# Vill-Lab/2023-TIFS-ISTVT

Measured on AMD Instinct MI355X. Metric: clips/sec (BxTx3x224x224 fwd+bwd), higher is better.
Workload: dtype bf16; 1 GPU; C2: B=32/GPU T=8 224x224 full ISTVT (Xception stem + 12-layer DSTTr) train step (fwd+bwd+grad all-reduce+SGD), random-init weights; global_batch=32, frames=8, size=224, depth=12, parallelism=dp1, early_allreduce=False, attn_fp8=False, dead_row_elimination=False, final_norm_class_rows_only=False, optimizer=SGD(momentum 0.9) fused, step_graphs=False

## Files before the change

### 2023-tifs-istvt_amd/_lib.py

```python
import ctypes
import os
from ctypes import c_float, c_int, c_long, c_void_p

_HERE = os.path.dirname(os.path.abspath(__file__))
LIB_PATH = os.environ.get('ISTVT_LIB') or os.path.join(_HERE, 'libistvt_hip.so')

P, I, L, F = c_void_p, c_int, c_long, c_float


class JpegDecodeArgs(ctypes.Structure):
    _fields_ = [('bytes', P), ('nbytes', L), ('images', P), ('images_host', P), ('segments', P), ('segments_host', P),
                ('qtabs', P), ('htabs', P), ('scratch', P), ('scratch_bytes', L), ('out', P), ('sizes', P), ('status', P),
                ('stream', P), ('n', I), ('nseg', I), ('nq', I), ('nh', I), ('Hc', I), ('Wc', I)]


class JpegEncodeArgs(ctypes.Structure):
    _fields_ = [('frames', P), ('total', L), ('quality', P), ('header', P), ('header_bytes', L), ('scratch', P),
                ('scratch_bytes', L), ('data', P), ('capacity', L), ('offsets', P), ('status', P), ('stream', P), ('n', I),
                ('H', I), ('W', I), ('subsampling', I), ('restart_interval', I), ('dqt0', I), ('dqt1', I)]


SIGNATURES = {
    'istvt_gemm': [P, L, I, P, L, I, P, L, I, I, I, P, P, L, P, I, I, I, F, P, P, I, I, P],
    'istvt_layernorm_fwd': [P, L, P, P, P, L, P, P, L, I, F, I, P],
# ... 11 lines not shown
    'istvt_attn_spatial_relevance': [P, L, P, L, P, P, P, I, I, I, I, F, I, P],
    'istvt_attn_temporal_relevance': [P, L, P, L, P, P, I, I, I, I, I, F, I, I, P],
    'istvt_relevance_heatmap': [P, P, I, I, I, P],
    'istvt_relevance_fuse_windows': [P, P, P, P, P, P, P, P, P, I, I, I, I, I, I, P],
    'istvt_relevance_overlay_u8': [P, P, P, P, P, I, I, I, I, P],
    'istvt_windows_reduce': [P, P, P, P, I, I, I, P],
    'istvt_auc_pairs': [P, P, F, P, L, P, P, I, P],
    'istvt_tokens_fwd': [P, P, P, P, P, L, I, I, I, I, I, I, P],
    'istvt_tokens_gather_fwd': [P, P, P, P, P, P, L, I, I, I, I, I, I, I, P],
    'istvt_tokens_bwd': [P, L, P, P, P, P, P, I, I, I, I, I, I, P],
    'istvt_frame_diff': [P, P, I, I, I, I, I, I, P],
    'istvt_stats_replicas': [],
    'istvt_stats_reduce': [P, I, P],
    'istvt_stats_reduce_add': [P, I, P, P],
    'istvt_bn_stats': [P, P, P, L, I, I, P],
    'istvt_bn_finalize': [P, P, ctypes.c_double, P, P, P, P, F, F, P, I, I, I, P],
    'istvt_bn_apply': [P, P, P, L, I, I, I, P],
    'istvt_bn_bwd_stats': [P, P, P, P, P, L, I, I, P],
    'istvt_bn_bwd_apply': [P, P, P, P, P, P, P, P, P, L, I, I, I, P],
    'istvt_bn_add_fwd': [P, P, P, P, P, L, I, I, P],
    'istvt_pw_bwd': [P, P, P, P, P, P, P, L, P, L, P, P, P, P, P, L, I, I, I, I, P],
    'istvt_pw_bwd_grid': [L],
    'istvt_pw_bwd_rows': [],
    'istvt_im2col_conv1': [P, P, I, I, I, P],
    'istvt_conv1_fwd': [P, P, P, I, I, I, P],
    'istvt_conv1_fwd_u8': [P, P, P, P, P, I, I, I, P],
    'istvt_conv1_wgrad': [P, P, P, P, I, I, I, P],
    'istvt_conv1_wgrad_slabs': [],
    'istvt_conv1_fwd_u8_view': [P, L, I, I, P, P, P, P, P, I, I, I, P],
    'istvt_conv1_wgrad_u8': [P, P, L, I, I, P, P, P, P, P, I, I, I, P],
    'istvt_im2col_conv1_u8': [P, L, I, I, P, P, P, P, I, I, I, P],
    'istvt_crop_resize_u8': [P, L, I, I, P, P, I, I, P],
    'istvt_crop_resize_nv12': [P, L, I, I, L, L, P, P, P, I, I, P],
    'istvt_nv12_to_rgb_u8': [P, L, I, I, L, L, P, P, I, P],
    'istvt_warp_similarity_u8': [P, L, I, I, P, P, I, I, P],
    'istvt_warp_similarity_nv12': [P, L, I, I, L, L, P, P, P, I, I, P],
    'istvt_relevance_paste_u8': [P, L, I, I, P, I, P, P, P, P, I, I, P],
    'istvt_relevance_paste_nv12': [P, L, I, I, L, L, P, I, P, P, P, P, I, I, P],
    'istvt_jpeg_roundtrip_u8': [P, L, I, I, I, P, I, P, L, P, P],
    'istvt_jpeg_decode_u8': [ctypes.POINTER(JpegDecodeArgs)],
    'istvt_jpeg_decode_split_u8': [ctypes.POINTER(JpegDecodeArgs), I],
    'istvt_jpeg_decode_indexed_u8': [ctypes.POINTER(JpegDecodeArgs), I, I, I, I, I],
    'istvt_jpeg_decode_indexed_split_u8': [ctypes.POINTER(JpegDecodeArgs), I, I, I, I, I, I, I, I],
    'istvt_batch_draw': [ctypes.POINTER(JpegDecodeArgs), I, I, I],
    'istvt_jpeg_decode_drawn_u8': [ctypes.POINTER(JpegDecodeArgs), I, I, I, I, I, I, I],
    'istvt_jpeg_decode_drawn_split_u8': [ctypes.POINTER(JpegDecodeArgs), I, I, I, I, I, I, I, I, I, I],
# ... 88 lines not shown
```

### 2023-tifs-istvt_amd/csrc/pw_bwd.hip

```cpp
#include "common.h"
#include "bn_bwd.h"

constexpr int PW_R = 128;
constexpr int PW_THREADS = 512;

__host__ __device__ constexpr int pw_lds_row(int p) { return (p & ~31) | ((p & 4) << 2) | ((p & 24) >> 1) | (p & 3); }

static inline int pw_bwd_split(long M, long* kper_out) {
    long splits = M / 512 < 1 ? 1 : (M / 512 > 256 ? 256 : M / 512);
    if (splits > (M + 63) / 64) splits = (M + 63) / 64;
    long kper = (M + splits - 1) / splits;
    kper = (kper + 63) / 64 * 64;
    if (kper_out) *kper_out = kper;
    return (int)((M + kper - 1) / kper);
}

template <int CIN, int COUT>
struct PwTile {
    static constexpr int NU = PW_R * (COUT / 8) / PW_THREADS;
    static constexpr int ND = PW_R * (CIN / 8) / PW_THREADS;
    bf16x8 dz[NU], u[NU], d[ND];
};

template <int CIN, int COUT>
__global__ __launch_bounds__(PW_THREADS) void pw_bwd_kernel(
    const bf16_t* __restrict__ dz, const bf16_t* __restrict__ u, const float* __restrict__ bnp,
    const float* __restrict__ gamma, const double* s1, const double* s2, const bf16_t* __restrict__ d, long ldd,
    const bf16_t* __restrict__ wt, long ldwt, bf16_t* __restrict__ dd, float* __restrict__ ws, float* dgamma,
    float* dbeta, long M, long kper, int batch_stats) {
    static_assert(COUT == 128 && (CIN == 64 || CIN == 128), "instantiated shapes");
    constexpr int LDU = COUT + 16, LDD = CIN + 16;
    constexpr int UCH = COUT / 8, DCH = CIN / 8;
    constexpr int UROWS = PW_THREADS / UCH, DROWS = PW_THREADS / DCH;
    constexpr int KT = CIN / 16, KS = COUT / 32;
    constexpr int MT = (PW_R / 16) * KT / 8;
    typedef PwTile<CIN, COUT> Tile;
    __shared__ __attribute__((aligned(16))) bf16_t s_du[PW_R * LDU];
    __shared__ __attribute__((aligned(16))) bf16_t s_d[PW_R * LDD];
    __shared__ __attribute__((aligned(16))) bf16_t s_dd[PW_R * LDD];
    __shared__ __attribute__((aligned(16))) BnBwdChunk s_kc[UCH];

    const int tid = threadIdx.x, lane = tid & 63;
    const int wave = __builtin_amdgcn_readfirstlane(tid >> 6);
    const int g = lane >> 4, r = lane & 15;
    const long row_begin = (long)blockIdx.x * kper;
    const long row_end = min(M, row_begin + kper);
    const long nblk = (row_end - row_begin + PW_R - 1) / PW_R;

    const int uc = tid % UCH, ur = tid / UCH;
    const int dc = tid % DCH, dr = tid / DCH;
    const float invM = batch_stats ? 1.0f / (float)M : 0.0f;
    if (tid < UCH) bn_bwd_chunk_load(s_kc[tid], bnp, gamma, s1, s2, COUT, tid * 8, invM);
    __syncthreads();

    const int kt_dd = wave % KT, mt0 = (wave / KT) * MT;
    bf16x8 wf[KS];
#pragma unroll
    for (int s = 0; s < KS; ++s)
        wf[s] = *reinterpret_cast<const bf16x8*>(wt + (long)(kt_dd * 16 + r) * ldwt + s * 32 + g * 8);

    f32x4 accw[KT];
#pragma unroll
    for (int kt = 0; kt < KT; ++kt) accw[kt] = f32x4{0.f, 0.f, 0.f, 0.f};

    constexpr unsigned OOB = 0x80000000u, RSRC_FLAGS = 0x00020000u;
    const __amdgpu_buffer_rsrc_t dz_rs = __builtin_amdgcn_make_buffer_rsrc((void*)dz, 0, (int)(row_end * COUT * 2), RSRC_FLAGS);
    const __amdgpu_buffer_rsrc_t u_rs = __builtin_amdgcn_make_buffer_rsrc((void*)u, 0, (int)(row_end * COUT * 2), RSRC_FLAGS);
    const __amdgpu_buffer_rsrc_t d_rs = __builtin_amdgcn_make_buffer_rsrc((void*)d, 0, (int)(row_end * ldd * 2), RSRC_FLAGS);
    const __amdgpu_buffer_rsrc_t dd_rs = __builtin_amdgcn_make_buffer_rsrc((void*)dd, 0, (int)(row_end * CIN * 2), RSRC_FLAGS);
    const int ldd2 = (int)ldd * 2;

    auto load = [&](Tile& t, const long b) {
        const long row0 = row_begin + b * PW_R;
#pragma unroll
        for (int i = 0; i < Tile::NU; ++i) {
            const long row = row0 + ur + i * UROWS;
            const unsigned off = row < row_end ? (unsigned)((int)row * (COUT * 2) + uc * 16) : OOB;
            t.dz[i] = __builtin_bit_cast(bf16x8, __builtin_amdgcn_raw_buffer_load_b128(dz_rs, off, 0, 0));
            t.u[i] = __builtin_bit_cast(bf16x8, __builtin_amdgcn_raw_buffer_load_b128(u_rs, off, 0, 0));
        }
#pragma unroll
        for (int i = 0; i < Tile::ND; ++i) {
            const long row = row0 + dr + i * DROWS;
            const unsigned off = row < row_end ? (unsigned)((int)row * ldd2 + dc * 16) : OOB;
            t.d[i] = __builtin_bit_cast(bf16x8, __builtin_amdgcn_raw_buffer_load_b128(d_rs, off, 0, 0));
        }
    };

    auto block = [&](Tile& t, const long b, const long bnext) {
        const long row0 = row_begin + b * PW_R;
        const BnBwdChunk kc = s_kc[uc];
#pragma unroll
        for (int i = 0; i < Tile::NU; ++i) {
            const int lr = ur + i * UROWS;
            const unsigned keep = row0 + lr < row_end ? 0xffffffffu : 0u;
            bf16x8 o;
#pragma unroll
            for (int j = 0; j < 8; ++j) o[j] = (bf16_t)bn_bwd_du((float)t.dz[i][j], (float)t.u[i][j], kc, j);
            *reinterpret_cast<u32x4*>(s_du + pw_lds_row(lr) * LDU + uc * 8) = __builtin_bit_cast(u32x4, o) & keep;
        }
#pragma unroll
        for (int i = 0; i < Tile::ND; ++i)
            *reinterpret_cast<bf16x8*>(s_d + pw_lds_row(dr + i * DROWS) * LDD + dc * 8) = t.d[i];
        load(t, bnext);
        __syncthreads();
#pragma unroll
        for (int mt = 0; mt < MT; ++mt) {
            const int m = (mt0 + mt) * 16 + r;
            f32x4 acc = f32x4{0.f, 0.f, 0.f, 0.f};
#pragma unroll
            for (int s = 0; s < KS; ++s) {
                const bf16x8 bu = *reinterpret_cast<const bf16x8*>(s_du + m * LDU + s * 32 + g * 8);
                acc = __builtin_amdgcn_mfma_f32_16x16x32_bf16(wf[s], bu, acc, 0, 0, 0);
            }
            bf16x4 o;
#pragma unroll
            for (int e = 0; e < 4; ++e) o[e] = (bf16_t)acc[e];
            *reinterpret_cast<bf16x4*>(s_dd + m * LDD + kt_dd * 16 + g * 4) = o;
        }
#pragma unroll
        for (int s = 0; s < PW_R / 32; ++s) {
            const int ka = s * 32 + g * 4, kb = ka + 16;
            const bf16x8 bu = frag_load_tr(s_du, LDU, ka, kb, wave * 16, r);
#pragma unroll
            for (int kt = 0; kt < KT; ++kt) {
                const bf16x8 ad = frag_load_tr(s_d, LDD, ka, kb, kt * 16, r);
                accw[kt] = __builtin_amdgcn_mfma_f32_16x16x32_bf16(ad, bu, accw[kt], 0, 0, 0);
            }
        }
        __syncthreads();
#pragma unroll
        for (int i = 0; i < Tile::ND; ++i) {
            const int lr = dr + i * DROWS;
            const long row = row0 + lr;
            const unsigned off = row < row_end ? (unsigned)((int)row * (CIN * 2) + dc * 16) : OOB;
            __builtin_amdgcn_raw_buffer_store_b128(*reinterpret_cast<const u32x4*>(s_dd + pw_lds_row(lr) * LDD + dc * 8), dd_rs,
                                                   off, 0, 0);
        }
    };

    Tile t0, t1;
    load(t0, 0);
    __builtin_amdgcn_sched_barrier(0);
    load(t1, 1);
    __builtin_amdgcn_sched_barrier(0);
    for (long b = 0; b < nblk; b += 2) {
        block(t0, b, b + 2);
        block(t1, b + 1, b + 3);
    }

    float* slab = ws + (long)blockIdx.x * (COUT * CIN);
#pragma unroll
    for (int kt = 0; kt < KT; ++kt)
        *reinterpret_cast<f32x4*>(slab + (wave * 16 + r) * CIN + kt * 16 + g * 4) = accw[kt];

    if (blockIdx.x == 0) {
        for (int c = tid; c < COUT; c += PW_THREADS) {
            if (dgamma) dgamma[c] += (float)s2[c];
            if (dbeta) dbeta[c] += (float)s1[c];
        }
    }
}

extern "C" int istvt_pw_bwd_grid(long M) { return M > 0 ? pw_bwd_split(M, nullptr) : 0; }
extern "C" int istvt_pw_bwd_rows() { return PW_R; }

extern "C" int istvt_pw_bwd(const void* dz, const void* u, const float* bnp, const float* gamma, const double* s1,
                            const double* s2, const void* d, long ldd, const void* wt, long ldwt, void* dd, float* ws,
                            float* wgrad_out, float* dgamma, float* dbeta, long M, int Cin, int Cout, int batch_stats,
                            int dtype, hipStream_t stream) {
    if (dtype != DT_BF16) return ISTVT_ERR_DTYPE;
    if (M <= 0 || Cout != 128 || (Cin != 64 && Cin != 128)) return ISTVT_ERR_SHAPE;
    if (ldd < Cin || ldd % 8 != 0 || ldwt < Cout || ldwt % 8 != 0) return ISTVT_ERR_SHAPE;
    if (M * Cout * 2 >= 0x7fffffffL || M * ldd * 2 >= 0x7fffffffL) return ISTVT_ERR_SHAPE;
    if (!dz || !u || !bnp || !gamma || !s1 || !s2 || !d || !wt || !dd || !ws || !wgrad_out) return ISTVT_ERR_SHAPE;
    long kper = 0;
    const int G = pw_bwd_split(M, &kper);
#define PW_LAUNCH(CI, CO)                                                                                              \
    hipLaunchKernelGGL((pw_bwd_kernel<CI, CO>), dim3((unsigned)G), dim3(PW_THREADS), 0, stream, (const bf16_t*)dz,      \
                       (const bf16_t*)u, bnp, gamma, s1, s2, (const bf16_t*)d, ldd, (const bf16_t*)wt, ldwt,           \
                       (bf16_t*)dd, ws, dgamma, dbeta, M, kper, batch_stats)
    if (Cin == 64) PW_LAUNCH(64, 128);
    else PW_LAUNCH(128, 128);
#undef PW_LAUNCH
    const int rc = istvt_check_launch();
    if (rc != ISTVT_OK) return rc;
    return istvt_splitk_reduce(ws, G, (long)Cout * Cin, wgrad_out, stream);
}
```

### 2023-tifs-istvt_amd/ops.py

```python
from __future__ import annotations

import os
from typing import Optional

import torch

from . import _lib
from ._common import (G256_MIN, ROW_ALIGN, Tensor, _DT, _c, _ptr, _req, _stream, cast, dtype_code,
                      empty_rows, pad_ld, rows, zeros_rows)
from .frames import (batch_draw, crop_resize_nv12, crop_resize_u8, decode_frames, draw_clips, encode_frames,
                     jpeg_bank_ingest, jpeg_decode_drawn_u8, jpeg_decode_indexed_u8, jpeg_decode_u8, jpeg_encode_u8,
                     jpeg_roundtrip_u8, nv12_to_rgb_u8, perturb_u8, png_decode_u8, relevance_paste_nv12, relevance_paste_u8,
                     warp_similarity_nv12, warp_similarity_u8)
from .weights import (_refresh_derived, _refresh_plain_copies, _static_holders, _transposed_operand,
                      _versions, derived, invalidate_weight_cache, refresh_stale_operands, set_static_addresses,
                      static_addresses, weight_as, weight_cat_as)


gemm_profile = None
kernel_profile = None


class prof:

# ... 194 lines not shown
        kper = -(-(-(-M // splits)) // 64) * 64
        splits = -(-M // kper)
        ws = torch.empty((splits, N, K), dtype=torch.float32, device=dy.device)
        gemm_raw(dy, ldy, False, x, ldx, False, ws, K, N, K, M, out_mode=3, splitk=splits)
        _lib.check(_lib.lib().istvt_splitk_reduce(ws.data_ptr(), splits, N * K, out.data_ptr(), _stream()),
                   'istvt_splitk_reduce')
    elif splits > 1:
        bk = 64 if dy.dtype == torch.bfloat16 else 32
        kper = -(-(-(-M // splits)) // bk) * bk
        splits = -(-M // kper)
        ws = torch.empty((splits, N, K), dtype=torch.float32, device=dy.device)
        gemm_raw(dy, ldy, False, x, ldx, False, ws, K, N, K, M, out_mode=3, splitk=splits)
        if (N * K) % 4 == 0:
            _lib.check(_lib.lib().istvt_splitk_reduce(ws.data_ptr(), splits, N * K, out.data_ptr(), _stream()),
                       'istvt_splitk_reduce')
        else:
            _lib.check(_lib.lib().istvt_rows_reduce(ws.data_ptr(), splits, N * K, out.data_ptr(), _stream()), 'istvt_rows_reduce')
    else:
        gemm_raw(dy, ldy, False, x, ldx, False, out, K, N, K, M, out_mode=2, splitk=1)
    return out


PW_BWD_PAIRS = ((64, 128), (128, 128))


def pw_bwd_geometry(M: int):
    lib = _lib.lib()
    return int(lib.istvt_pw_bwd_grid(M)), int(lib.istvt_pw_bwd_rows())


def pw_bwd_fusable(dz: Tensor, d: Tensor, w: Tensor) -> bool:
    if dz.dtype != torch.bfloat16 or d.dtype != torch.bfloat16 or w.dtype != torch.bfloat16:
        return False
    if dz.dim() != 2 or d.dim() != 2 or w.dim() != 2 or not dz.is_contiguous() or not d.is_contiguous():
        return False
    M, cout = dz.shape
    cin = d.shape[1]
    if d.shape[0] != M or tuple(w.shape) != (cout, cin) or (cin, cout) not in PW_BWD_PAIRS or M < 1:
        return False
    return M * cout * 2 < 0x7fffffff and dz.data_ptr() % 16 == 0 and d.data_ptr() % 16 == 0


def pw_bwd(dz: Tensor, u: Tensor, bnp: Tensor, gamma: Tensor, stats: Tensor, d: Tensor, w: Tensor, out: Tensor,
           dgamma: Tensor, dbeta: Tensor, training: bool = True) -> Tensor:
    for t in (dz, u, d, w, out, dgamma, dbeta):
        _req(t)
    M, cout = dz.shape
    cin = d.shape[1]
    if u.shape != dz.shape or not u.is_contiguous() or u.dtype != dz.dtype:
        raise RuntimeError('pw_bwd: u must match dz (%s %s vs %s %s)' % (tuple(u.shape), u.dtype, tuple(dz.shape), dz.dtype))
    if out.dtype != torch.float32 or out.numel() != cout * cin or not out.is_contiguous():
        raise RuntimeError('pw_bwd: the weight gradient must be contiguous float32 [%d, %d]' % (cout, cin))
    wt, ldwt = rows(_transposed_operand(w))
    lib = _lib.lib()
    G = int(lib.istvt_pw_bwd_grid(M))
    dd = torch.empty((M, cin), dtype=dz.dtype, device=dz.device)
    ws = torch.empty((G, cout * cin), dtype=torch.float32, device=dz.device)
    with prof('pw_bwd_fused', (2 * M * cout + 2 * M * cin) * dz.element_size()):
        _lib.check(lib.istvt_pw_bwd(dz.data_ptr(), u.data_ptr(), bnp.data_ptr(), gamma.data_ptr(), stats[0, 0].data_ptr(),
                                    stats[0, 1].data_ptr(), d.data_ptr(), d.stride(0), wt.data_ptr(), ldwt, dd.data_ptr(),
                                    ws.data_ptr(), out.data_ptr(), dgamma.data_ptr(), dbeta.data_ptr(), M, cin, cout,
                                    int(training), dtype_code(dz), _stream()), 'istvt_pw_bwd')
    return dd


WGRAD_GROUP_MAX = 8


def wgrad_groupable(dy: Tensor, x: Tensor) -> bool:
    if dy.dtype != torch.bfloat16 or x.dtype != torch.bfloat16 or dy.dim() != 2 or x.dim() != 2:
        return False
    M, N = dy.shape
    K = x.shape[1]
    if N < G256_MIN or K < G256_MIN or N % 8 or K % 8 or x.shape[0] != M:
        return False
    for t in (dy, x):
        if t.stride(1) != 1 or (t.stride(0) * 2) % 16 or t.data_ptr() % 16 or M * t.stride(0) * 2 >= 0x7fffffff:
            return False
    return True


def linear_wgrad_group(items) -> None:
    import ctypes as C
    n = len(items)
    if not 1 <= n <= WGRAD_GROUP_MAX:
# ... 694 lines not shown
```

### 2023-tifs-istvt_amd/parallel.py

```python
from __future__ import annotations

import itertools
import operator
import os
import weakref
from typing import Iterable, List, Tuple

import torch
import torch.distributed as dist

from . import stem as _stem


def _single_rank(group=None) -> bool:
    return dist.get_world_size(group) == 1 and os.environ.get('ISTVT_FORCE_COLLECTIVES') != '1'


def live_named_parameters(model: torch.nn.Module) -> List[Tuple[str, torch.nn.Parameter]]:
    keep = set('xcep.model.' + n for n in _stem.param_names())
    out = []
    for name, p in model.named_parameters():
        if not p.requires_grad:
            continue
        if name.startswith('xcep.') and name not in keep:
# ... 488 lines not shown
        from . import functional as Fn
        entry, ctx.entry, ctx.token = ctx.entry, None, None
        entry.static_gout.copy_(g)
        cur = torch.cuda.current_stream(g.device)
        side = Fn._overlap['streams'].get(g.device.index)
        if side is not None:
            cur.wait_stream(side)
        entry.g_bwd.replay()
        if side is not None:
            side.wait_stream(cur)
        return None, None, None


class _GraphEntry:
    __slots__ = ('static_x', 'static_out', 'static_gout', 'g_fwd', 'g_bwd', 'keep', 'fingerprint', 'live', 'calls', 'pool')


def env_switches() -> tuple:
    env = os.environ.get
    return (env('ISTVT_STEM_MATERIALISE_A2', '0') == '1', env('ISTVT_STEM_WGRAD_SIDE', '1') != '0',
            env('ISTVT_STEM_PW_BWD_FUSED', '1') != '0', env('ISTVT_BGRAD_SIDE', '0') == '1')


_training_of = operator.attrgetter('training')


class ModuleIndex:

    def __init__(self, model: torch.nn.Module):
        keep = set('xcep.model.' + n for n in _stem.param_names())
        mods, self.slots = [], []
        for prefix, mod in model.named_modules():
            mods.append(mod)
            for leaf in mod._parameters:
                name = prefix + '.' + leaf if prefix else leaf
                if name.startswith('xcep.') and name not in keep:
                    continue
                self.slots.append((mod._parameters, leaf))
        self._child_dicts = [mod._modules for mod in mods]
        self._param_dicts = [mod._parameters for mod in mods]
        self._children = self._walk()
        self._param_count = sum(map(len, self._param_dicts))
        self._root = weakref.ref(model)
        self.modules = mods[1:]
        self.dropouts = [mod for mod in self.modules if isinstance(mod, torch.nn.Dropout)]
        self.fp8 = [mod for mod in self.modules if hasattr(mod, 'attn_fp8')]
# ... 39 lines not shown
        ops._static_holders.add(self)

    def forward_eager(self, x):
        return self._fwd()(x)

    def note_eager(self, reason: str):
        self.last_reason = reason
        self.stats['eager'] += 1

    def index(self) -> ModuleIndex:
        idx = self._tree
        if idx is None or idx.stale():
            if idx is not None:
                if self.entries:
                    self.stats['recaptures'] += 1
                self.drop()
            idx = self._tree = ModuleIndex(self.model())
        return idx

    def _config(self, m):
        from . import functional as Fn
        if m is None:
            return None
        return (str(getattr(m, 'compute_dtype', None)), self.index().flags(), env_switches(), bool(Fn._overlap['on']),
                int(Fn._overlap['group']), bool(Fn.GELU_SAVE_DERIV[0]), os.environ.get('ISTVT_GEMM_TM', ''))

    def key(self, x, grads: bool):
        m = self.model()
        return (tuple(x.shape), x.dtype, x.device.index, self._config(m), bool(m is not None and m.training), bool(grads))

    def live_parameters(self):
        self.live = self.index().live()
        return self.live

    def _live(self):
        return self.live if self.live is not None else self.live_parameters()

    def _fingerprint(self, grads: bool, live=None):
        fp = []
        for p in (self._live() if live is None else live):
            fp.append(id(p))
            fp.append(p.data_ptr())
            if grads:
                g = p.grad
                if g is None or not getattr(p, '_istvt_fused_grad', False):
                    return None
                fp.append(g.data_ptr())
# ... 132 lines not shown
```

### 2023-tifs-istvt_amd/stem.py

```python
from __future__ import annotations

from typing import List, Optional

import os

import torch
from torch.autograd import Function
from torch.autograd.function import once_differentiable

from . import _lib, ops
from .ops import _c, _ptr, _req, _stream, dtype_code

Tensor = torch.Tensor
BN_EPS = 1e-5
BN_MOMENTUM = 0.1


def out_side(side: int) -> int:
    s = (side - 3) // 2 + 1 - 2
    for _ in range(3):
        s = (s - 1) // 2 + 1
    return s


# ... 96 lines not shown

def _bn_backward_apply(dz: Tensor, u: Tensor, st: BNState, gamma: Tensor, M: int, C: int, stats: Tensor, dg: Tensor,
                       db: Tensor, training: bool) -> Tensor:
    du = torch.empty_like(u)
    with ops.prof('bn_bwd_apply', 3 * M * C * u.element_size()):
        _lib.check(_lib.lib().istvt_bn_bwd_apply(dz.data_ptr(), u.data_ptr(), st.ptr(), gamma.data_ptr(),
                                                 stats[0, 0].data_ptr(), stats[0, 1].data_ptr(), du.data_ptr(), dg.data_ptr(),
                                                 db.data_ptr(), M, C, int(training), dtype_code(u), _stream()),
                   'istvt_bn_bwd_apply')
    return du


def _bn_backward_sums(dz: Tensor, u: Tensor, st: BNState, M: int, C: int, stats: Optional[Tensor]) -> Tensor:
    if stats is None:
        stats = new_stats(C, u.device)
        with ops.prof('bn_bwd_stats', 2 * M * C * u.element_size()):
            _lib.check(_lib.lib().istvt_bn_bwd_stats(dz.data_ptr(), u.data_ptr(), st.ptr(), stats[0, 0].data_ptr(),
                                                     stats[0, 1].data_ptr(), M, C, dtype_code(u), _stream()),
                       'istvt_bn_bwd_stats')
    reduce_stats(stats, C)
    return stats


def pointwise_bn_backward(dz: Tensor, u: Tensor, st: BNState, gamma: Tensor, M: int, cout: int, d: Tensor, w: Tensor,
                          cin: int, stats: Optional[Tensor], dg: Tensor, db: Tensor, wgrad_target: Optional[Tensor],
                          training: bool, side=None):
    stats = _bn_backward_sums(dz, u, st, M, cout, stats)
    if os.environ.get('ISTVT_STEM_PW_BWD_FUSED', '1') != '0' and ops.pw_bwd_fusable(dz, d, w):
        dW = None
        if wgrad_target is None:
            dW = wgrad_target = torch.zeros((cout, cin), dtype=torch.float32, device=dz.device)
        dd = ops.pw_bwd(dz, u, st.pack, gamma, stats, d, w, wgrad_target, dg, db, training)
        return dd, dW
    du = _bn_backward_apply(dz, u, st, gamma, M, cout, stats, dg, db, training)
    dW = None
    if wgrad_target is not None and side is not None:
        side(lambda: ops.linear_wgrad(du, d, out=wgrad_target), (du, d))
    else:
        r = ops.linear_wgrad(du, d, out=wgrad_target)
        dW = r if wgrad_target is None else None
    return ops.linear_dgrad(du, w, blocked=False), dW


def dwconv(x: Tensor, w9: Tensor, Fr: int, H: int, W: int, C: int, *, in_bn: Optional[BNState] = None,
           in_relu: bool = False, flip: bool = False, msrc: Optional[Tensor] = None, m_bn: Optional[BNState] = None,
           mask_pre: bool = False, mask_post: bool = False, addsrc: Optional[Tensor] = None,
           stats: Optional[Tensor] = None) -> Tensor:
    out = torch.empty((Fr * H * W, C), dtype=x.dtype, device=x.device)
    Ha, Wa = (H - 1) // 2 + 1, (W - 1) // 2 + 1
    nel = Fr * H * W * C
    nbytes = (2 * nel + (nel if msrc is not None else 0) + (nel // 4 if addsrc is not None else 0)) * x.element_size()
    with ops.prof('dwconv3x3', nbytes, 18.0 * nel):
        _lib.check(_lib.lib().istvt_dwconv3x3(
            x.data_ptr(), w9.data_ptr(), out.data_ptr(), Fr, H, W, C,
            in_bn.ptr() if in_bn else None, int(in_relu), int(flip),
# ... 208 lines not shown
            if tg is None:
                grads[n + '.weight'] = dg
            if tb is None:
                grads[n + '.bias'] = db
            return du

        side_on = os.environ.get('ISTVT_STEM_WGRAD_SIDE', '1') != '0'

        def lin_wgrad(n, dyv, xv):
            q = P[n]
            t = tgt(n, (q.shape[0], -1))
            if t is not None and side_on:
                from . import functional as Fn
                Fn.side_launch(dyv.device, lambda: ops.linear_wgrad(dyv, xv, out=t), keep=(dyv, xv))
                return
            r = ops.linear_wgrad(dyv, xv, out=t)
            if t is None:
                grads[n] = r

        def side_wgrad(fn, keep):
            from . import functional as Fn
            Fn.side_launch(keep[0].device, fn, keep=keep)

        def pw_bn_bwd(dz, u, st, nbn, M_, C_, d, wp, nw, cin_, stats):
            q = P[nw]
            tg, tb, t = tgt(nbn + '.weight', (C_,)), tgt(nbn + '.bias', (C_,)), tgt(nw, (q.shape[0], -1))
            dg = tg if tg is not None else torch.zeros((C_,), dtype=torch.float32, device=u.device)
            db = tb if tb is not None else torch.zeros((C_,), dtype=torch.float32, device=u.device)
            dd, dW = pointwise_bn_backward(dz, u, st, P[nbn + '.weight'], M_, C_, d, wp, cin_, stats, dg, db, t, training,
                                           side=side_wgrad if side_on else None)
            if tg is None:
                grads[nbn + '.weight'] = dg
            if tb is None:
                grads[nbn + '.bias'] = db
            if t is None:
                grads[nw] = dW
            return dd

        def dw_wgrad(n, xv, dv, H_, C_, bn_, relu_):
            t = tgt(n, (C_, 9))
            if t is not None and side_on:
                from . import functional as Fn
                Fn.side_launch(dv.device, lambda: dwconv_wgrad(xv, dv, Fr, H_, H_, C_, bn_, relu_, out=t), keep=(xv, dv, bn_))
                return
            r = dwconv_wgrad(xv, dv, Fr, H_, H_, C_, bn_, relu_, out=t)
            if t is None:
                grads[n] = r

        dOut = _c(dy).reshape(-1, 728)
        for blk in reversed(sv['blocks']):
            name, i0, cin, cout, H, Hs = blk['name'], blk['i0'], blk['cin'], blk['cout'], blk['H'], blk['Hs']
            M, Ms = Fr * H * H, Fr * Hs * Hs
            dev = dOut.device
            duS = bn_bwd(dOut, blk['uS'], blk['bnS'], name + '.skipbn', Ms, cout)
            lin_wgrad(name + '.skip.weight', duS, blk['xs'])
            dxs = ops.linear_dgrad(duS, blk['wsk'], blocked=False)
            dzB = torch.empty((M, cout), dtype=dtype, device=dev)
            statsB = new_stats(cout, dev) if training else None
            with ops.prof('pool_bwd', ((2 if training else 1) * M + Ms) * cout * dzB.element_size() + Ms * cout):
                _lib.check(L.istvt_pool_bwd(dOut.data_ptr(), blk['amax'].data_ptr(), dzB.data_ptr(), Fr, H, H, cout,
                                            blk['uB'].data_ptr() if training else None, blk['bnB'].ptr() if training else None,
                                            statsB[0, 0].data_ptr() if training else None,
                                            statsB[0, 1].data_ptr() if training else None, dtc, _stream()), 'istvt_pool_bwd')
            sB = '%s.rep.%d' % (name, i0 + 3)
            dd2 = pw_bn_bwd(dzB, blk['uB'], blk['bnB'], '%s.rep.%d' % (name, i0 + 4), M, cout, blk['d2'], blk['wpwB'],
                            sB + '.pointwise.weight', cout, statsB)
            del dzB
            dw_wgrad(sB + '.conv1.weight', blk['uA'], dd2, H, cout, blk['bnA'], True)
            statsA = new_stats(cout, dev)
            dzA = dwconv(dd2, blk['wdwB'], Fr, H, H, cout, flip=True, msrc=blk['uA'], m_bn=blk['bnA'], mask_pre=True,
                         stats=statsA)
            del dd2
            sA = '%s.rep.%d' % (name, i0)
            dd1 = pw_bn_bwd(dzA, blk['uA'], blk['bnA'], '%s.rep.%d' % (name, i0 + 1), M, cout, blk['d1'], blk['wpwA'],
                            sA + '.pointwise.weight', cin, statsA)
            del dzA
            fused_in = not blk['pre_relu'] and blk['X'] is sv['u2']
            dw_wgrad(sA + '.conv1.weight', blk['X'], dd1, H, cin, sv['bn2'] if fused_in else None, True if fused_in else blk['pre_relu'])
            if blk['pre_relu']:
# ... 136 lines not shown
```

### 2023-tifs-istvt_amd/xblocks.py

```python
from __future__ import annotations

from typing import List, Optional, Sequence, Tuple

import torch
from torch.autograd import Function
from torch.autograd.function import once_differentiable

from . import _lib, ops
from . import stem as _stem
from .ops import _c, _req, _stream, dtype_code
from .stem import (bn_apply, bn_backward, bn_forward_stats, dwconv, dwconv_wgrad, new_stats, pointwise_bn,
                   pointwise_bn_backward)

Tensor = torch.Tensor


def nhwc(x: Tensor) -> Tensor:
    return _c(x.permute(0, 2, 3, 1))


def nchw_view(y: Tensor) -> Tensor:
    return y.permute(0, 3, 1, 2)


def _tap_major(w: Tensor) -> Tensor:
    return _stem.tap_major(w)


def _fused_target(q: Tensor, shape):
    if getattr(q, '_istvt_fused_grad', False) and q.grad is not None and q.grad.is_contiguous():
        return q.grad.view(shape)
    return None


class SepConvFn(Function):
# ... 112 lines not shown
        dtype, dev = dout.dtype, dout.device
        dtc = dtype_code(dout)
        nu = len(units)
        M = Fr * H * W
        grads: List[Optional[Tensor]] = [None] * len(params)

        def bn_bwd(dz, u, st, gi, Mx, C, stats=None):
            g, b = params[gi], params[gi + 1]
            tg, tb = _fused_target(g, (C,)), _fused_target(b, (C,))
            du, dg, db = bn_backward(dz, u, st, g, Mx, C, stats=stats, dg=tg, db=tb, training=training)
            grads[gi] = None if tg is not None else dg
            grads[gi + 1] = None if tb is not None else db
            return du

        def lin_wgrad(wi, dyv, xv):
            q = params[wi]
            t = _fused_target(q, (q.shape[0], -1))
            r = ops.linear_wgrad(dyv, xv, out=t)
            grads[wi] = None if t is not None else r.view(q.shape)

        dskip, skip_full = None, False
        if spec.has_skip:
            Ms = Fr * sk['Hs'] * sk['Ws']
            duS = bn_bwd(dout, sk['uS'], sk['bnS'], 4 * nu + 1, Ms, spec.cout)
            lin_wgrad(4 * nu, duS, sk['xs'])
            if ctx.need_dx:
                dskip = ops.linear_dgrad(duS, sk['ws'], blocked=False)
                skip_full = spec.tail != 'pool'
        elif spec.tail == 'add':
            dskip, skip_full = dout, True
        if spec.tail == 'pool':
            dz = torch.empty((M, spec.cout), dtype=dtype, device=dev)
            last = units[nu - 1]
            stats = new_stats(spec.cout, dev) if training else None
            _lib.check(L.istvt_pool_bwd(dout.data_ptr(), sv['amax'].data_ptr(), dz.data_ptr(), Fr, H, W, spec.cout,
                                        last['u'].data_ptr() if training else None, last['bn'].ptr() if training else None,
                                        stats[0, 0].data_ptr() if training else None,
                                        stats[0, 1].data_ptr() if training else None, dtc, _stream()), 'istvt_pool_bwd')
        else:
            dz = dout
            stats = None
        dinp = None
        for i in reversed(range(nu)):
            un = units[i]
            cin, cout = un['cin'], un['cout']
            gq, bq, wq = params[4 * i + 2], params[4 * i + 3], params[4 * i + 1]
            tg, tb, tw = _fused_target(gq, (cout,)), _fused_target(bq, (cout,)), _fused_target(wq, (wq.shape[0], -1))
            dg = tg if tg is not None else torch.zeros((cout,), dtype=torch.float32, device=dev)
            db = tb if tb is not None else torch.zeros((cout,), dtype=torch.float32, device=dev)
            dd, dW = pointwise_bn_backward(dz, un['u'], un['bn'], gq, M, cout, un['d'], un['wp'], cin, stats, dg, db, tw,
# ... 54 lines not shown
```

### include/istvt_hip.h

```cpp
#ifndef ISTVT_HIP_H
#define ISTVT_HIP_H

#ifdef __cplusplus
extern "C" {
#endif

typedef struct ihipStream_t* istvt_stream_t;

#define ISTVT_OK 0
#define ISTVT_ERR_DTYPE (-2)
#define ISTVT_ERR_SHAPE (-3)
#define ISTVT_ERR_LAUNCH (-4)

#define ISTVT_F32 0
#define ISTVT_BF16 1

#define ISTVT_G256_MIN 64
int istvt_gemm(const void* A, long lda, int a_kc, const void* B, long ldb, int b_kc, void* C, long ldc, int M, int N,
               int K, const float* bias, const void* residual, long ldr, void* C2, int epi, int out_mode, int splitk,
               float alpha, double* col_sum, double* col_sumsq, int flags, int dtype, istvt_stream_t stream);

int istvt_splitk_reduce(const float* ws, int splits, long n, float* out, istvt_stream_t stream);

int istvt_wgrad_group(int count, const void* const* dy, const long* lddy, const void* const* x, const long* ldx,
// ... 56 lines not shown
                            istvt_stream_t stream);
int istvt_tokens_bwd(const void* dx, long lddx, void* dfeats, float* dspace, float* dtemporal, float* dpos, float* ws,
                     int B, int F, int P, int D, int pos_rows, int dtype, istvt_stream_t stream);

int istvt_frame_diff(const void* x, void* out, int B, int F, int P, int D, int adjoint, int dtype,
                     istvt_stream_t stream);


int istvt_stats_replicas(void);
int istvt_stats_reduce(double* acc, int C, istvt_stream_t stream);
int istvt_stats_reduce_add(const double* acc, int C, float* out, istvt_stream_t stream);

int istvt_bn_stats(const void* x, double* sum, double* sumsq, long M, int C, int dtype, istvt_stream_t stream);
int istvt_bn_finalize(const double* sum, const double* sumsq, double count, const float* gamma, const float* beta,
                      float* running_mean, float* running_var, float momentum, float eps, float* bnp, int C,
                      int use_batch, int update_running, istvt_stream_t stream);
int istvt_bn_apply(const void* x, const float* bnp, void* y, long M, int C, int relu, int dtype,
                   istvt_stream_t stream);
int istvt_bn_bwd_stats(const void* dz, const void* u, const float* bnp, double* s1, double* s2, long M, int C,
                       int dtype, istvt_stream_t stream);
int istvt_bn_bwd_apply(const void* dz, const void* u, const float* bnp, const float* gamma, const double* s1,
                       const double* s2, void* du, float* dgamma, float* dbeta, long M, int C, int batch_stats,
                       int dtype, istvt_stream_t stream);
int istvt_pw_bwd(const void* dz, const void* u, const float* bnp, const float* gamma, const double* s1, const double* s2,
                 const void* d, long ldd, const void* wt, long ldwt, void* dd, float* ws, float* wgrad_out,
                 float* dgamma, float* dbeta, long M, int Cin, int Cout, int batch_stats, int dtype,
                 istvt_stream_t stream);
int istvt_pw_bwd_grid(long M);
int istvt_pw_bwd_rows(void);
int istvt_bn_add_fwd(const void* x, const float* bnx, const void* skip, const float* bns, void* out, long M, int C,
                     int dtype, istvt_stream_t stream);

int istvt_im2col_conv1(const float* x, void* col, int frames, int S, int dtype, istvt_stream_t stream);
int istvt_col2im_conv1(const void* dcol, float* dx, int frames, int S, int dtype, istvt_stream_t stream);
int istvt_im2col3x3(const void* src, const float* bnp, int relu, void* col, int frames, int H, int W, int C,
                    int dtype, istvt_stream_t stream);
int istvt_col2im3x3(const void* dcol, const void* u, const float* bnp, void* dz, int frames, int H, int W, int C,
                    int dtype, istvt_stream_t stream);

int istvt_conv1_fwd(const float* x, const float* w, void* u1, int frames, int S, int dtype, istvt_stream_t stream);
int istvt_conv1_fwd_u8(const void* x, const float* mean, const float* std, const float* w, void* u1, int frames, int S,
                       int dtype, istvt_stream_t stream);
int istvt_conv1_wgrad(const void* du1, const float* x, float* slabs, float* dw, int frames, int S, int dtype,
                      istvt_stream_t stream);
int istvt_conv1_wgrad_slabs(void);
int istvt_conv1_fwd_u8_view(const void* x, long total, int Hs, int Ws, const int* view, const float* mean,
                            const float* std, const float* w, void* u1, int frames, int S, int dtype, istvt_stream_t stream);
int istvt_conv1_wgrad_u8(const void* du1, const void* x, long total, int Hs, int Ws, const int* view, const float* mean,
                         const float* std, float* slabs, float* dw, int frames, int S, int dtype, istvt_stream_t stream);
int istvt_im2col_conv1_u8(const void* x, long total, int Hs, int Ws, const int* view, const float* mean, const float* std,
                          void* col, int frames, int S, int dtype, istvt_stream_t stream);
int istvt_crop_resize_u8(const void* frames, long total, int Hs, int Ws, const int* boxes, void* out, int n, int S,
// ... 179 lines not shown
```

Baseline: 635.3 clips/s.

## Fuse skip-branch BN backward, wgrad and dgrad into pointwise kernel with wide variant

```diff
diff --git a/2023-tifs-istvt_amd/_lib.py b/2023-tifs-istvt_amd/_lib.py
--- a/2023-tifs-istvt_amd/_lib.py
+++ b/2023-tifs-istvt_amd/_lib.py
@@ -57,6 +57,7 @@
     'istvt_pw_bwd': [P, P, P, P, P, P, P, L, P, L, P, P, P, P, P, L, I, I, I, I, P],
     'istvt_pw_bwd_grid': [L],
     'istvt_pw_bwd_rows': [],
+    'istvt_pw_bwd_wide_rows': [],
     'istvt_im2col_conv1': [P, P, I, I, I, P],
     'istvt_conv1_fwd': [P, P, P, I, I, I, P],
     'istvt_conv1_fwd_u8': [P, P, P, P, P, I, I, I, P],
diff --git a/2023-tifs-istvt_amd/csrc/pw_bwd.hip b/2023-tifs-istvt_amd/csrc/pw_bwd.hip
--- a/2023-tifs-istvt_amd/csrc/pw_bwd.hip
+++ b/2023-tifs-istvt_amd/csrc/pw_bwd.hip
@@ -2,6 +2,7 @@
 #include "bn_bwd.h"
 
 constexpr int PW_R = 128;
+constexpr int PW_R_WIDE = 64;
 constexpr int PW_THREADS = 512;
 
 __host__ __device__ constexpr int pw_lds_row(int p) { return (p & ~31) | ((p & 4) << 2) | ((p & 24) >> 1) | (p & 3); }
@@ -15,53 +16,68 @@
     return (int)((M + kper - 1) / kper);
 }
 
-template <int CIN, int COUT>
+template <int CIN, int COUT, int R>
 struct PwTile {
-    static constexpr int NU = PW_R * (COUT / 8) / PW_THREADS;
-    static constexpr int ND = PW_R * (CIN / 8) / PW_THREADS;
+    static constexpr int NU = R * (COUT / 8) / PW_THREADS;
+    static constexpr int ND = R * (CIN / 8) / PW_THREADS;
     bf16x8 dz[NU], u[NU], d[ND];
 };
 
-template <int CIN, int COUT>
+template <int CIN, int COUT, int R>
 __global__ __launch_bounds__(PW_THREADS) void pw_bwd_kernel(
     const bf16_t* __restrict__ dz, const bf16_t* __restrict__ u, const float* __restrict__ bnp,
     const float* __restrict__ gamma, const double* s1, const double* s2, const bf16_t* __restrict__ d, long ldd,
     const bf16_t* __restrict__ wt, long ldwt, bf16_t* __restrict__ dd, float* __restrict__ ws, float* dgamma,
     float* dbeta, long M, long kper, int batch_stats) {
-    static_assert(COUT == 128 && (CIN == 64 || CIN == 128), "instantiated shapes");
+    static_assert((COUT == 128 && (CIN == 64 || CIN == 128) && R == PW_R) || (COUT == 256 && CIN == 128 && R == PW_R_WIDE),
+                  "instantiated shapes");
     constexpr int LDU = COUT + 16, LDD = CIN + 16;
     constexpr int UCH = COUT / 8, DCH = CIN / 8;
     constexpr int UROWS = PW_THREADS / UCH, DROWS = PW_THREADS / DCH;
     constexpr int KT = CIN / 16, KS = COUT / 32;
-    constexpr int MT = (PW_R / 16) * KT / 8;
-    typedef PwTile<CIN, COUT> Tile;
-    __shared__ __attribute__((aligned(16))) bf16_t s_du[PW_R * LDU];
-    __shared__ __attribute__((aligned(16))) bf16_t s_d[PW_R * LDD];
-    __shared__ __attribute__((aligned(16))) bf16_t s_dd[PW_R * LDD];
+    constexpr int MT = (R / 16) * KT / 8;
+    constexpr int OT = COUT / 128;
+    typedef PwTile<CIN, COUT, R> Tile;
+    __shared__ __attribute__((aligned(16))) bf16_t s_du[R * LDU];
+    __shared__ __attribute__((aligned(16))) bf16_t s_d[R * LDD];
+    __shared__ __attribute__((aligned(16))) bf16_t s_dd[R * LDD];
     __shared__ __attribute__((aligned(16))) BnBwdChunk s_kc[UCH];
+    constexpr bool W_LDS = COUT == 256;
+    __shared__ __attribute__((aligned(16))) bf16_t s_w[W_LDS ? CIN * LDU : 8];
 
     const int tid = threadIdx.x, lane = tid & 63;
     const int wave = __builtin_amdgcn_readfirstlane(tid >> 6);
     const int g = lane >> 4, r = lane & 15;
     const long row_begin = (long)blockIdx.x * kper;
     const long row_end = min(M, row_begin + kper);
-    const long nblk = (row_end - row_begin + PW_R - 1) / PW_R;
+    const long nblk = (row_end - row_begin + R - 1) / R;
 
     const int uc = tid % UCH, ur = tid / UCH;
     const int dc = tid % DCH, dr = tid / DCH;
     const float invM = batch_stats ? 1.0f / (float)M : 0.0f;
     if (tid < UCH) bn_bwd_chunk_load(s_kc[tid], bnp, gamma, s1, s2, COUT, tid * 8, invM);
+    if constexpr (W_LDS) {
+#pragma unroll
+        for (int i = 0; i < CIN * UCH / PW_THREADS; ++i) {
+            const int ch = tid + i * PW_THREADS, row = ch / UCH, c8 = (ch % UCH) * 8;
+            *reinterpret_cast<bf16x8*>(s_w + row * LDU + c8) = *reinterpret_cast<const bf16x8*>(wt + (long)row * ldwt + c8);
+        }
+    }
     __syncthreads();
 
     const int kt_dd = wave % KT, mt0 = (wave / KT) * MT;
     bf16x8 wf[KS];
-#pragma unroll
-    for (int s = 0; s < KS; ++s)
-        wf[s] = *reinterpret_cast<const bf16x8*>(wt + (long)(kt_dd * 16 + r) * ldwt + s * 32 + g * 8);
-
-    f32x4 accw[KT];
-#pragma unroll
-    for (int kt = 0; kt < KT; ++kt) accw[kt] = f32x4{0.f, 0.f, 0.f, 0.f};
+    if constexpr (!W_LDS) {
+#pragma unroll
+        for (int s = 0; s < KS; ++s)
+            wf[s] = *reinterpret_cast<const bf16x8*>(wt + (long)(kt_dd * 16 + r) * ldwt + s * 32 + g * 8);
+    }
+
+    f32x4 accw[OT][KT];
+#pragma unroll
+    for (int o = 0; o < OT; ++o)
+#pragma unroll
+        for (int kt = 0; kt < KT; ++kt) accw[o][kt] = f32x4{0.f, 0.f, 0.f, 0.f};
 
     constexpr unsigned OOB = 0x80000000u, RSRC_FLAGS = 0x00020000u;
     const __amdgpu_buffer_rsrc_t dz_rs = __builtin_amdgcn_make_buffer_rsrc((void*)dz, 0, (int)(row_end * COUT * 2), RSRC_FLAGS);
@@ -71,7 +87,7 @@
     const int ldd2 = (int)ldd * 2;
 
     auto load = [&](Tile& t, const long b) {
-        const long row0 = row_begin + b * PW_R;
+        const long row0 = row_begin + b * R;
 #pragma unroll
         for (int i = 0; i < Tile::NU; ++i) {
             const long row = row0 + ur + i * UROWS;
@@ -88,7 +104,7 @@
     };
 
     auto block = [&](Tile& t, const long b, const long bnext) {
-        const long row0 = row_begin + b * PW_R;
+        const long row0 = row_begin + b * R;
         const BnBwdChunk kc = s_kc[uc];
 #pragma unroll
         for (int i = 0; i < Tile::NU; ++i) {
@@ -104,6 +120,11 @@
             *reinterpret_cast<bf16x8*>(s_d + pw_lds_row(dr + i * DROWS) * LDD + dc * 8) = t.d[i];
         load(t, bnext);
         __syncthreads();
+        if constexpr (W_LDS) {
+#pragma unroll
+            for (int s = 0; s < KS; ++s)
+                wf[s] = *reinterpret_cast<const bf16x8*>(s_w + (kt_dd * 16 + r) * LDU + s * 32 + g * 8);
+        }
 #pragma unroll
         for (int mt = 0; mt < MT; ++mt) {
             const int m = (mt0 + mt) * 16 + r;
@@ -119,13 +140,17 @@
             *reinterpret_cast<bf16x4*>(s_dd + m * LDD + kt_dd * 16 + g * 4) = o;
         }
 #pragma unroll
-        for (int s = 0; s < PW_R / 32; ++s) {
+        for (int s = 0; s < R / 32; ++s) {
             const int ka = s * 32 + g * 4, kb = ka + 16;
-            const bf16x8 bu = frag_load_tr(s_du, LDU, ka, kb, wave * 16, r);
+            bf16x8 bu[OT];
+#pragma unroll
+            for (int o = 0; o < OT; ++o) bu[o] = frag_load_tr(s_du, LDU, ka, kb, (wave * OT + o) * 16, r);
 #pragma unroll
             for (int kt = 0; kt < KT; ++kt) {
                 const bf16x8 ad = frag_load_tr(s_d, LDD, ka, kb, kt * 16, r);
-                accw[kt] = __builtin_amdgcn_mfma_f32_16x16x32_bf16(ad, bu, accw[kt], 0, 0, 0);
+#pragma unroll
+                for (int o = 0; o < OT; ++o)
+                    accw[o][kt] = __builtin_amdgcn_mfma_f32_16x16x32_bf16(ad, bu[o], accw[o][kt], 0, 0, 0);
             }
         }
         __syncthreads();
@@ -151,8 +176,10 @@
 
     float* slab = ws + (long)blockIdx.x * (COUT * CIN);
 #pragma unroll
-    for (int kt = 0; kt < KT; ++kt)
-        *reinterpret_cast<f32x4*>(slab + (wave * 16 + r) * CIN + kt * 16 + g * 4) = accw[kt];
+    for (int o = 0; o < OT; ++o)
+#pragma unroll
+        for (int kt = 0; kt < KT; ++kt)
+            *reinterpret_cast<f32x4*>(slab + ((wave * OT + o) * 16 + r) * CIN + kt * 16 + g * 4) = accw[o][kt];
 
     if (blockIdx.x == 0) {
         for (int c = tid; c < COUT; c += PW_THREADS) {
@@ -164,24 +191,29 @@
 
 extern "C" int istvt_pw_bwd_grid(long M) { return M > 0 ? pw_bwd_split(M, nullptr) : 0; }
 extern "C" int istvt_pw_bwd_rows() { return PW_R; }
+extern "C" int istvt_pw_bwd_wide_rows() { return PW_R_WIDE; }
 
 extern "C" int istvt_pw_bwd(const void* dz, const void* u, const float* bnp, const float* gamma, const double* s1,
                             const double* s2, const void* d, long ldd, const void* wt, long ldwt, void* dd, float* ws,
-                            float* wgrad_out, float* dgamma, float* dbeta, long M, int Cin, int Cout, int batch_stats,
+                            float* wgrad_out, float* dgamma, float* dbeta, long M, int Cin, int Cout, int flags,
                             int dtype, hipStream_t stream) {
     if (dtype != DT_BF16) return ISTVT_ERR_DTYPE;
-    if (M <= 0 || Cout != 128 || (Cin != 64 && Cin != 128)) return ISTVT_ERR_SHAPE;
+    const bool wide = (flags & ISTVT_PW_BWD_WIDE) && Cout == 256 && Cin == 128;
+    if (M <= 0 || (flags & ~(ISTVT_PW_BWD_BATCH_STATS | ISTVT_PW_BWD_WIDE))) return ISTVT_ERR_SHAPE;
+    if (!wide && (Cout != 128 || (Cin != 64 && Cin != 128))) return ISTVT_ERR_SHAPE;
     if (ldd < Cin || ldd % 8 != 0 || ldwt < Cout || ldwt % 8 != 0) return ISTVT_ERR_SHAPE;
     if (M * Cout * 2 >= 0x7fffffffL || M * ldd * 2 >= 0x7fffffffL) return ISTVT_ERR_SHAPE;
     if (!dz || !u || !bnp || !gamma || !s1 || !s2 || !d || !wt || !dd || !ws || !wgrad_out) return ISTVT_ERR_SHAPE;
     long kper = 0;
     const int G = pw_bwd_split(M, &kper);
-#define PW_LAUNCH(CI, CO)                                                                                              \
-    hipLaunchKernelGGL((pw_bwd_kernel<CI, CO>), dim3((unsigned)G), dim3(PW_THREADS), 0, stream, (const bf16_t*)dz,      \
+    const int batch_stats = flags & ISTVT_PW_BWD_BATCH_STATS;
+#define PW_LAUNCH(CI, CO, R)                                                                                           \
+    hipLaunchKernelGGL((pw_bwd_kernel<CI, CO, R>), dim3((unsigned)G), dim3(PW_THREADS), 0, stream, (const bf16_t*)dz,   \
                        (const bf16_t*)u, bnp, gamma, s1, s2, (const bf16_t*)d, ldd, (const bf16_t*)wt, ldwt,           \
                        (bf16_t*)dd, ws, dgamma, dbeta, M, kper, batch_stats)
-    if (Cin == 64) PW_LAUNCH(64, 128);
-    else PW_LAUNCH(128, 128);
+    if (wide) PW_LAUNCH(128, 256, PW_R_WIDE);
+    else if (Cin == 64) PW_LAUNCH(64, 128, PW_R);
+    else PW_LAUNCH(128, 128, PW_R);
 #undef PW_LAUNCH
     const int rc = istvt_check_launch();
     if (rc != ISTVT_OK) return rc;
diff --git a/2023-tifs-istvt_amd/ops.py b/2023-tifs-istvt_amd/ops.py
--- a/2023-tifs-istvt_amd/ops.py
+++ b/2023-tifs-istvt_amd/ops.py
@@ -240,27 +240,30 @@
 
 
 PW_BWD_PAIRS = ((64, 128), (128, 128))
-
-
-def pw_bwd_geometry(M: int):
+PW_BWD_WIDE_PAIRS = ((128, 256),)
+PW_BWD_FLAG_WIDE = 2
+
+
+def pw_bwd_geometry(M: int, wide: bool = False):
     lib = _lib.lib()
-    return int(lib.istvt_pw_bwd_grid(M)), int(lib.istvt_pw_bwd_rows())
-
-
-def pw_bwd_fusable(dz: Tensor, d: Tensor, w: Tensor) -> bool:
+    return int(lib.istvt_pw_bwd_grid(M)), int(lib.istvt_pw_bwd_wide_rows() if wide else lib.istvt_pw_bwd_rows())
+
+
+def pw_bwd_fusable(dz: Tensor, d: Tensor, w: Tensor, wide: bool = False) -> bool:
     if dz.dtype != torch.bfloat16 or d.dtype != torch.bfloat16 or w.dtype != torch.bfloat16:
         return False
     if dz.dim() != 2 or d.dim() != 2 or w.dim() != 2 or not dz.is_contiguous() or not d.is_contiguous():
         return False
     M, cout = dz.shape
     cin = d.shape[1]
-    if d.shape[0] != M or tuple(w.shape) != (cout, cin) or (cin, cout) not in PW_BWD_PAIRS or M < 1:
+    pairs = PW_BWD_WIDE_PAIRS if wide else PW_BWD_PAIRS
+    if d.shape[0] != M or tuple(w.shape) != (cout, cin) or (cin, cout) not in pairs or M < 1:
         return False
     return M * cout * 2 < 0x7fffffff and dz.data_ptr() % 16 == 0 and d.data_ptr() % 16 == 0
 
 
 def pw_bwd(dz: Tensor, u: Tensor, bnp: Tensor, gamma: Tensor, stats: Tensor, d: Tensor, w: Tensor, out: Tensor,
-           dgamma: Tensor, dbeta: Tensor, training: bool = True) -> Tensor:
+           dgamma: Tensor, dbeta: Tensor, training: bool = True, wide: bool = False) -> Tensor:
     for t in (dz, u, d, w, out, dgamma, dbeta):
         _req(t)
     M, cout = dz.shape
@@ -278,7 +281,8 @@
         _lib.check(lib.istvt_pw_bwd(dz.data_ptr(), u.data_ptr(), bnp.data_ptr(), gamma.data_ptr(), stats[0, 0].data_ptr(),
                                     stats[0, 1].data_ptr(), d.data_ptr(), d.stride(0), wt.data_ptr(), ldwt, dd.data_ptr(),
                                     ws.data_ptr(), out.data_ptr(), dgamma.data_ptr(), dbeta.data_ptr(), M, cin, cout,
-                                    int(training), dtype_code(dz), _stream()), 'istvt_pw_bwd')
+                                    int(training) | (PW_BWD_FLAG_WIDE if wide else 0), dtype_code(dz), _stream()),
+                   'istvt_pw_bwd')
     return dd
 
 
diff --git a/2023-tifs-istvt_amd/parallel.py b/2023-tifs-istvt_amd/parallel.py
--- a/2023-tifs-istvt_amd/parallel.py
+++ b/2023-tifs-istvt_amd/parallel.py
@@ -534,6 +534,10 @@
             env('ISTVT_STEM_PW_BWD_FUSED', '1') != '0', env('ISTVT_BGRAD_SIDE', '0') == '1')
 
 
+def env_switch_pw_bwd_wide() -> bool:
+    return os.environ.get('ISTVT_STEM_PW_BWD_WIDE', '1') != '0'
+
+
 _training_of = operator.attrgetter('training')
 
 
@@ -619,7 +623,8 @@
         from . import functional as Fn
         if m is None:
             return None
-        return (str(getattr(m, 'compute_dtype', None)), self.index().flags(), env_switches(), bool(Fn._overlap['on']),
+        return (str(getattr(m, 'compute_dtype', None)), self.index().flags(), env_switches(), env_switch_pw_bwd_wide(),
+                bool(Fn._overlap['on']),
                 int(Fn._overlap['group']), bool(Fn.GELU_SAVE_DERIV[0]), os.environ.get('ISTVT_GEMM_TM', ''))
 
     def key(self, x, grads: bool):
diff --git a/2023-tifs-istvt_amd/stem.py b/2023-tifs-istvt_amd/stem.py
--- a/2023-tifs-istvt_amd/stem.py
+++ b/2023-tifs-istvt_amd/stem.py
@@ -142,15 +142,28 @@
     return stats
 
 
+def pw_bwd_wide_on() -> bool:
+    return os.environ.get('ISTVT_STEM_PW_BWD_WIDE', '1') != '0'
+
+
+def pw_bwd_skip_fusable(dz: Tensor, d: Tensor, w: Tensor) -> bool:
+    return pw_bwd_wide_on() and (ops.pw_bwd_fusable(dz, d, w) or ops.pw_bwd_fusable(dz, d, w, wide=True))
+
+
 def pointwise_bn_backward(dz: Tensor, u: Tensor, st: BNState, gamma: Tensor, M: int, cout: int, d: Tensor, w: Tensor,
                           cin: int, stats: Optional[Tensor], dg: Tensor, db: Tensor, wgrad_target: Optional[Tensor],
-                          training: bool, side=None):
+                          training: bool, side=None, skip: bool = False):
     stats = _bn_backward_sums(dz, u, st, M, cout, stats)
-    if os.environ.get('ISTVT_STEM_PW_BWD_FUSED', '1') != '0' and ops.pw_bwd_fusable(dz, d, w):
+    wide = ops.pw_bwd_fusable(dz, d, w, wide=True)
+    if skip or wide:
+        take = pw_bwd_wide_on() and (wide or ops.pw_bwd_fusable(dz, d, w))
+    else:
+        take = os.environ.get('ISTVT_STEM_PW_BWD_FUSED', '1') != '0' and ops.pw_bwd_fusable(dz, d, w)
+    if take:
         dW = None
         if wgrad_target is None:
             dW = wgrad_target = torch.zeros((cout, cin), dtype=torch.float32, device=dz.device)
-        dd = ops.pw_bwd(dz, u, st.pack, gamma, stats, d, w, wgrad_target, dg, db, training)
+        dd = ops.pw_bwd(dz, u, st.pack, gamma, stats, d, w, wgrad_target, dg, db, training, wide=wide)
         return dd, dW
     du = _bn_backward_apply(dz, u, st, gamma, M, cout, stats, dg, db, training)
     dW = None
@@ -405,13 +418,13 @@
             from . import functional as Fn
             Fn.side_launch(keep[0].device, fn, keep=keep)
 
-        def pw_bn_bwd(dz, u, st, nbn, M_, C_, d, wp, nw, cin_, stats):
+        def pw_bn_bwd(dz, u, st, nbn, M_, C_, d, wp, nw, cin_, stats, skip=False):
             q = P[nw]
             tg, tb, t = tgt(nbn + '.weight', (C_,)), tgt(nbn + '.bias', (C_,)), tgt(nw, (q.shape[0], -1))
             dg = tg if tg is not None else torch.zeros((C_,), dtype=torch.float32, device=u.device)
             db = tb if tb is not None else torch.zeros((C_,), dtype=torch.float32, device=u.device)
             dd, dW = pointwise_bn_backward(dz, u, st, P[nbn + '.weight'], M_, C_, d, wp, cin_, stats, dg, db, t, training,
-                                           side=side_wgrad if side_on else None)
+                                           side=side_wgrad if side_on else None, skip=skip)
             if tg is None:
                 grads[nbn + '.weight'] = dg
             if tb is None:
@@ -435,9 +448,14 @@
             name, i0, cin, cout, H, Hs = blk['name'], blk['i0'], blk['cin'], blk['cout'], blk['H'], blk['Hs']
             M, Ms = Fr * H * H, Fr * Hs * Hs
             dev = dOut.device
-            duS = bn_bwd(dOut, blk['uS'], blk['bnS'], name + '.skipbn', Ms, cout)
-            lin_wgrad(name + '.skip.weight', duS, blk['xs'])
-            dxs = ops.linear_dgrad(duS, blk['wsk'], blocked=False)
+            if pw_bwd_skip_fusable(dOut, blk['xs'], blk['wsk']):
+                dxs = pw_bn_bwd(dOut, blk['uS'], blk['bnS'], name + '.skipbn', Ms, cout, blk['xs'], blk['wsk'],
+                                name + '.skip.weight', cin, None, skip=True)
+            else:
+                duS = bn_bwd(dOut, blk['uS'], blk['bnS'], name + '.skipbn', Ms, cout)
+                lin_wgrad(name + '.skip.weight', duS, blk['xs'])
+                dxs = ops.linear_dgrad(duS, blk['wsk'], blocked=False)
+                del duS
             dzB = torch.empty((M, cout), dtype=dtype, device=dev)
             statsB = new_stats(cout, dev) if training else None
             with ops.prof('pool_bwd', ((2 if training else 1) * M + Ms) * cout * dzB.element_size() + Ms * cout):
diff --git a/2023-tifs-istvt_amd/xblocks.py b/2023-tifs-istvt_amd/xblocks.py
--- a/2023-tifs-istvt_amd/xblocks.py
+++ b/2023-tifs-istvt_amd/xblocks.py
@@ -10,7 +10,7 @@
 from . import stem as _stem
 from .ops import _c, _req, _stream, dtype_code
 from .stem import (bn_apply, bn_backward, bn_forward_stats, dwconv, dwconv_wgrad, new_stats, pointwise_bn,
-                   pointwise_bn_backward)
+                   pointwise_bn_backward, pw_bwd_skip_fusable)
 
 Tensor = torch.Tensor
 
@@ -169,10 +169,25 @@
         dskip, skip_full = None, False
         if spec.has_skip:
             Ms = Fr * sk['Hs'] * sk['Ws']
-            duS = bn_bwd(dout, sk['uS'], sk['bnS'], 4 * nu + 1, Ms, spec.cout)
-            lin_wgrad(4 * nu, duS, sk['xs'])
+            if pw_bwd_skip_fusable(dout, sk['xs'], sk['ws']):
+                gq, bq, wq = params[4 * nu + 1], params[4 * nu + 2], params[4 * nu]
+                tg, tb = _fused_target(gq, (spec.cout,)), _fused_target(bq, (spec.cout,))
+                tw = _fused_target(wq, (wq.shape[0], -1))
+                dg = tg if tg is not None else torch.zeros((spec.cout,), dtype=torch.float32, device=dev)
+                db = tb if tb is not None else torch.zeros((spec.cout,), dtype=torch.float32, device=dev)
+                dskip, dW = pointwise_bn_backward(dout, sk['uS'], sk['bnS'], gq, Ms, spec.cout, sk['xs'], sk['ws'], spec.cin,
+                                                  None, dg, db, tw, training, skip=True)
+                grads[4 * nu + 1] = None if tg is not None else dg
+                grads[4 * nu + 2] = None if tb is not None else db
+                grads[4 * nu] = None if tw is not None else dW.view(wq.shape)
+                if not ctx.need_dx:
+                    dskip = None
+            else:
+                duS = bn_bwd(dout, sk['uS'], sk['bnS'], 4 * nu + 1, Ms, spec.cout)
+                lin_wgrad(4 * nu, duS, sk['xs'])
+                if ctx.need_dx:
+                    dskip = ops.linear_dgrad(duS, sk['ws'], blocked=False)
             if ctx.need_dx:
-                dskip = ops.linear_dgrad(duS, sk['ws'], blocked=False)
                 skip_full = spec.tail != 'pool'
         elif spec.tail == 'add':
             dskip, skip_full = dout, True
diff --git a/include/istvt_hip.h b/include/istvt_hip.h
--- a/include/istvt_hip.h
+++ b/include/istvt_hip.h
@@ -102,12 +102,15 @@
 int istvt_bn_bwd_apply(const void* dz, const void* u, const float* bnp, const float* gamma, const double* s1,
                        const double* s2, void* du, float* dgamma, float* dbeta, long M, int C, int batch_stats,
                        int dtype, istvt_stream_t stream);
+#define ISTVT_PW_BWD_BATCH_STATS 1
+#define ISTVT_PW_BWD_WIDE 2
 int istvt_pw_bwd(const void* dz, const void* u, const float* bnp, const float* gamma, const double* s1, const double* s2,
                  const void* d, long ldd, const void* wt, long ldwt, void* dd, float* ws, float* wgrad_out,
-                 float* dgamma, float* dbeta, long M, int Cin, int Cout, int batch_stats, int dtype,
+                 float* dgamma, float* dbeta, long M, int Cin, int Cout, int flags, int dtype,
                  istvt_stream_t stream);
 int istvt_pw_bwd_grid(long M);
 int istvt_pw_bwd_rows(void);
+int istvt_pw_bwd_wide_rows(void);
 int istvt_bn_add_fwd(const void* x, const float* bnx, const void* skip, const float* bns, void* out, long M, int C,
                      int dtype, istvt_stream_t stream);
 
```

Result: no change. 638.7 clips/s, median of 6 (+0.5%).
